# grantneale/kafka-lag-based-assignor

Measured on AMD Instinct MI355X. Metric: partition-assignments/sec (whole node), higher is better.
Workload: dtype int64

## Files before the change

### kafka_lag_based_assignor_amd/csrc/la_sort32.h

```cpp
#pragma once
#include <hip/hip_runtime.h>
#include <stdint.h>

#include "la_device.h"
#include "la_sort64.h"

#ifndef LA_SORT32_MED3
#define LA_SORT32_MED3 1
#endif

namespace la {

template <int J>
__device__ __forceinline__ uint32_t dir_vec() {
    const uint32_t lane = __builtin_amdgcn_mbcnt_hi(~0u, __builtin_amdgcn_mbcnt_lo(~0u, 0u));
    return (lane & (uint32_t)J) ? 0xFFFFFFFFu : 0u;
}

#if LA_SORT32_MED3
#define LA32_SAME_ASM(PADSTR, CTRL)                                             \
    asm volatile(PADSTR                                                         \
                 "v_mov_b32_dpp %1, %0 " CTRL LA_DPP_TAIL "\n\t"                \
                 "v_med3_u32 %0, %0, %1, %2"                                    \
                 : "+v"(x), "=&v"(t1)                                           \
                 : "v"(dir))

#define LA32_SAME_PADS(CTRL)                                      \
    do {                                                          \
        if constexpr (PAD == 0) LA32_SAME_ASM(LA_PAD0, CTRL);      \
        else if constexpr (PAD == 1) LA32_SAME_ASM(LA_PAD1, CTRL); \
        else LA32_SAME_ASM(LA_PAD2, CTRL);                         \
    } while (0)

template <int J, int PAD>
__device__ __forceinline__ void cmpx32_same_xor(uint32_t& x) {
    const uint32_t dir = dir_vec<J>();
    uint32_t t1;
    if constexpr (J == 1) LA32_SAME_PADS("quad_perm:[1,0,3,2]");
    else if constexpr (J == 2) LA32_SAME_PADS("quad_perm:[2,3,0,1]");
    else if constexpr (J == 8) LA32_SAME_PADS("row_ror:8");
    else if constexpr (J == 4) {
        uint32_t h;
        asm volatile(LA_PAD2
                     "v_mov_b32_dpp %2, %0 row_half_mirror" LA_DPP_TAIL "\n\t"
                     "s_nop 1\n\t"
                     "v_mov_b32_dpp %1, %2 quad_perm:[3,2,1,0]" LA_DPP_TAIL "\n\t"
                     "v_med3_u32 %0, %0, %1, %3"
                     : "+v"(x), "=&v"(t1), "=&v"(h)
                     : "v"(dir));
    } else {
        uint32_t b;
        if constexpr (J == 16)
            asm volatile(LA_PAD2 "v_mov_b32 %1, %0\n\ts_nop 1\n\tv_permlane16_swap_b32 %0, %1\n\t"
                         "v_med3_u32 %0, %0, %1, %2"
                         : "+v"(x), "=&v"(b) : "v"(dir));
        else
            asm volatile(LA_PAD2 "v_mov_b32 %1, %0\n\ts_nop 1\n\tv_permlane32_swap_b32 %0, %1\n\t"
                         "v_med3_u32 %0, %0, %1, %2"
                         : "+v"(x), "=&v"(b) : "v"(dir));
    }
}

template <int M, int PAD>
__device__ __forceinline__ void cmpx32_same_mirror(uint32_t& x) {
    if constexpr (M == 2) {
        cmpx32_same_xor<1, PAD>(x);
    } else if constexpr (M == 4 || M == 8 || M == 16) {
        const uint32_t dir = dir_vec<M / 2>();
        uint32_t t1;
        if constexpr (M == 4) LA32_SAME_PADS("quad_perm:[3,2,1,0]");
        else if constexpr (M == 8) LA32_SAME_PADS("row_half_mirror");
        else LA32_SAME_PADS("row_mirror");
    } else {
        asm volatile("s_nop 1" : "+v"(x));
        const uint32_t o = shfl_mirror<M>(x);
        const bool keep_min = (KeepMin<M / 2>::value >> __lane_id()) & 1;
        const uint32_t lo = o < x ? o : x, hi = o < x ? x : o;
        x = keep_min ? lo : hi;
        asm volatile("s_nop 1" : "+v"(x));
    }
}

#define LA32_CROSS_ASM(PADSTR, CTRL)                                            \
    asm volatile(PADSTR                                                         \
                 "v_mov_b32_dpp %2, %1 " CTRL LA_DPP_TAIL "\n\t"                \
                 "v_mov_b32_dpp %3, %0 " CTRL LA_DPP_TAIL "\n\t"                \
                 "v_med3_u32 %0, %0, %2, %4\n\t"                               \
                 "v_med3_u32 %1, %1, %3, %4"                                    \
                 : "+v"(r), "+v"(q), "=&v"(t1), "=&v"(t2)                        \
                 : "v"(dir))

#define LA32_CROSS_PADS(CTRL)                                      \
    do {                                                           \
        if constexpr (PAD == 0) LA32_CROSS_ASM(LA_PAD0, CTRL);      \
        else if constexpr (PAD == 1) LA32_CROSS_ASM(LA_PAD1, CTRL); \
        else LA32_CROSS_ASM(LA_PAD2, CTRL);                         \
    } while (0)

template <int M, int PAD>
__device__ __forceinline__ void cmpx32_cross_mirror(uint32_t& r, uint32_t& q) {
    if constexpr (M <= 16) {
        const uint32_t dir = dir_vec<M / 2>();
        uint32_t t1, t2;
        if constexpr (M == 2) LA32_CROSS_PADS("quad_perm:[1,0,3,2]");
        else if constexpr (M == 4) LA32_CROSS_PADS("quad_perm:[3,2,1,0]");
        else if constexpr (M == 8) LA32_CROSS_PADS("row_half_mirror");
        else LA32_CROSS_PADS("row_mirror");
    } else {
        const uint64_t keep = KeepMin<M / 2>::value;
        asm volatile("s_nop 1" : "+v"(r), "+v"(q));
        const uint32_t oq = shfl_mirror<M>(q), orr = shfl_mirror<M>(r);
        const bool keep_min = (keep >> __lane_id()) & 1;
        const uint32_t rl = oq < r ? oq : r, rh = oq < r ? r : oq;
        const uint32_t ql = orr < q ? orr : q, qh = orr < q ? q : orr;
        r = keep_min ? rl : rh;
        q = keep_min ? ql : qh;
        asm volatile("s_nop 1" : "+v"(r), "+v"(q));
    }
}

#else

#define LA32_SAME_ASM(PADSTR, CTRL)                                             \
    asm volatile(PADSTR                                                         \
                 "v_min_u32_dpp %1, %0, %0 " CTRL LA_DPP_TAIL "\n\t"              \
                 "v_max_u32_dpp %2, %0, %0 " CTRL LA_DPP_TAIL "\n\t"              \
                 "v_cndmask_b32_e64 %0, %2, %1, %3"                             \
                 : "+v"(x), "=&v"(t1), "=&v"(t2)                                 \
                 : "s"(keep))

#define LA32_SAME_PADS(CTRL)                                      \
    do {                                                          \
        if constexpr (PAD == 0) LA32_SAME_ASM(LA_PAD0, CTRL);      \
        else if constexpr (PAD == 1) LA32_SAME_ASM(LA_PAD1, CTRL); \
        else LA32_SAME_ASM(LA_PAD2, CTRL);                         \
    } while (0)

template <int J, int PAD>
__device__ __forceinline__ void cmpx32_same_xor(uint32_t& x) {
    const uint64_t keep = KeepMin<J>::value;
    uint32_t t1, t2;
    if constexpr (J == 1) LA32_SAME_PADS("quad_perm:[1,0,3,2]");
    else if constexpr (J == 2) LA32_SAME_PADS("quad_perm:[2,3,0,1]");
    else if constexpr (J == 8) LA32_SAME_PADS("row_ror:8");
    else if constexpr (J == 4) {
        uint32_t h;
        asm volatile(LA_PAD2
                     "v_mov_b32_dpp %3, %0 row_half_mirror" LA_DPP_TAIL "\n\t"
                     "s_nop 1\n\t"
                     "v_min_u32_dpp %1, %3, %0 quad_perm:[3,2,1,0]" LA_DPP_TAIL "\n\t"
                     "v_max_u32_dpp %2, %3, %0 quad_perm:[3,2,1,0]" LA_DPP_TAIL "\n\t"
                     "v_cndmask_b32_e64 %0, %2, %1, %4"
                     : "+v"(x), "=&v"(t1), "=&v"(t2), "=&v"(h)
                     : "s"(keep));
    } else {
        uint32_t b;
        if constexpr (J == 16)
            asm volatile(LA_PAD2 "v_mov_b32 %3, %0\n\ts_nop 1\n\tv_permlane16_swap_b32 %0, %3\n\t"
                         "v_min_u32 %1, %0, %3\n\tv_max_u32 %2, %0, %3\n\tv_cndmask_b32_e64 %0, %2, %1, %4"
                         : "+v"(x), "=&v"(t1), "=&v"(t2), "=&v"(b) : "s"(keep));
        else
            asm volatile(LA_PAD2 "v_mov_b32 %3, %0\n\ts_nop 1\n\tv_permlane32_swap_b32 %0, %3\n\t"
                         "v_min_u32 %1, %0, %3\n\tv_max_u32 %2, %0, %3\n\tv_cndmask_b32_e64 %0, %2, %1, %4"
                         : "+v"(x), "=&v"(t1), "=&v"(t2), "=&v"(b) : "s"(keep));
    }
}

template <int M, int PAD>
__device__ __forceinline__ void cmpx32_same_mirror(uint32_t& x) {
    if constexpr (M == 2) {
        cmpx32_same_xor<1, PAD>(x);
    } else if constexpr (M == 4 || M == 8 || M == 16) {
        const uint64_t keep = KeepMin<M / 2>::value;
        uint32_t t1, t2;
        if constexpr (M == 4) LA32_SAME_PADS("quad_perm:[3,2,1,0]");
        else if constexpr (M == 8) LA32_SAME_PADS("row_half_mirror");
        else LA32_SAME_PADS("row_mirror");
    } else {
        asm volatile("s_nop 1" : "+v"(x));
        const uint32_t o = shfl_mirror<M>(x);
        const bool keep_min = (KeepMin<M / 2>::value >> __lane_id()) & 1;
        const uint32_t lo = o < x ? o : x, hi = o < x ? x : o;
        x = keep_min ? lo : hi;
        asm volatile("s_nop 1" : "+v"(x));
    }
}

#define LA32_CROSS_ASM(PADSTR, CTRL)                                            \
    asm volatile(PADSTR                                                         \
                 "v_min_u32_dpp %2, %1, %0 " CTRL LA_DPP_TAIL "\n\t"              \
                 "v_max_u32_dpp %3, %1, %0 " CTRL LA_DPP_TAIL "\n\t"              \
                 "v_min_u32_dpp %4, %0, %1 " CTRL LA_DPP_TAIL "\n\t"              \
                 "v_max_u32_dpp %5, %0, %1 " CTRL LA_DPP_TAIL "\n\t"              \
                 "v_cndmask_b32_e64 %0, %3, %2, %6\n\t"                         \
                 "v_cndmask_b32_e64 %1, %5, %4, %6"                             \
                 : "+v"(r), "+v"(q), "=&v"(t1), "=&v"(t2), "=&v"(t3), "=&v"(t4)  \
                 : "s"(keep))

#define LA32_CROSS_PADS(CTRL)                                      \
    do {                                                           \
        if constexpr (PAD == 0) LA32_CROSS_ASM(LA_PAD0, CTRL);      \
        else if constexpr (PAD == 1) LA32_CROSS_ASM(LA_PAD1, CTRL); \
        else LA32_CROSS_ASM(LA_PAD2, CTRL);                         \
    } while (0)

template <int M, int PAD>
__device__ __forceinline__ void cmpx32_cross_mirror(uint32_t& r, uint32_t& q) {
    const uint64_t keep = KeepMin<M / 2>::value;
    if constexpr (M <= 16) {
        uint32_t t1, t2, t3, t4;
        if constexpr (M == 2) LA32_CROSS_PADS("quad_perm:[1,0,3,2]");
        else if constexpr (M == 4) LA32_CROSS_PADS("quad_perm:[3,2,1,0]");
        else if constexpr (M == 8) LA32_CROSS_PADS("row_half_mirror");
        else LA32_CROSS_PADS("row_mirror");
    } else {
        asm volatile("s_nop 1" : "+v"(r), "+v"(q));
        const uint32_t oq = shfl_mirror<M>(q), orr = shfl_mirror<M>(r);
        const bool keep_min = (keep >> __lane_id()) & 1;
        const uint32_t rl = oq < r ? oq : r, rh = oq < r ? r : oq;
        const uint32_t ql = orr < q ? orr : q, qh = orr < q ? q : orr;
        r = keep_min ? rl : rh;
        q = keep_min ? ql : qh;
        asm volatile("s_nop 1" : "+v"(r), "+v"(q));
    }
}

#endif

__device__ __forceinline__ void cmpx32_regs(uint32_t& a, uint32_t& b) {
    const uint32_t lo = a < b ? a : b, hi = a < b ? b : a;
    a = lo;
    b = hi;
}

template <int L, int E, int J>
__device__ __forceinline__ void clean32(uint32_t (&key)[E]) {
    if constexpr (J >= 1) {
        if constexpr (J >= E) {
            constexpr int PADN = (E <= 2) ? 2 : 0;
#pragma unroll
            for (int r = 0; r < E; ++r) cmpx32_same_xor<J / E, PADN>(key[r]);
        } else {
#pragma unroll
            for (int r = 0; r < E; ++r)
                if ((r & J) == 0) cmpx32_regs(key[r], key[r | J]);
        }
        clean32<L, E, J / 2>(key);
    }
}

template <int L, int E, int K>
__device__ __forceinline__ void merge32(uint32_t (&key)[E]) {
    if constexpr (K <= L * E) {
        if constexpr (K <= E) {
#pragma unroll
            for (int r = 0; r < E; ++r)
                if ((r & (K >> 1)) == 0) cmpx32_regs(key[r], key[r ^ (K - 1)]);
        } else {
            constexpr int M = K / E;
            if constexpr (E == 1) {
                cmpx32_same_mirror<M, 2>(key[0]);
            } else {
#pragma unroll
                for (int r = E / 2 - 1; r >= 0; --r) cmpx32_cross_mirror<M, 2>(key[r], key[E - 1 - r]);
            }
        }
        clean32<L, E, K / 4>(key);
        merge32<L, E, K * 2>(key);
    }
}

template <int L, int E>
__device__ __forceinline__ void bitonic_sort_tile_u32(uint32_t (&key)[E]) {
    merge32<L, E, 2>(key);
}

}
```

### kafka_lag_based_assignor_amd/csrc/la_sort64.h

```cpp
#pragma once
#include <hip/hip_runtime.h>
#include <stdint.h>

#include "la_device.h"

namespace la {

struct P64 {
    uint32_t lo, hi;
};

__device__ __forceinline__ P64 p64_from(uint64_t x) { P64 p; p.lo = (uint32_t)x; p.hi = (uint32_t)(x >> 32); return p; }
__device__ __forceinline__ uint64_t p64_value(const P64& p) { return ((uint64_t)p.hi << 32) | p.lo; }

template <int J>
struct KeepMin {
    static_assert(J == 1 || J == 2 || J == 4 || J == 8 || J == 16 || J == 32, "bad lane bit");
    static constexpr uint64_t value = J == 1 ? 0x5555555555555555ull : J == 2 ? 0x3333333333333333ull
                                    : J == 4 ? 0x0F0F0F0F0F0F0F0Full : J == 8 ? 0x00FF00FF00FF00FFull
                                    : J == 16 ? 0x0000FFFF0000FFFFull : 0x00000000FFFFFFFFull;
};

#define LA_DPP_TAIL " row_mask:0xf bank_mask:0xf"
#define LA_FIX_S(K) "s_xor_b64 vcc, vcc, " K "\n\t"
#define LA_FIX_V(T, K) "v_xor_b32 " T ", " K ", " T "\n\t" "v_cmp_gt_i32 vcc, 0, " T "\n\t"

template <int J>
__device__ __forceinline__ uint32_t keep_vec() {
    const uint32_t lane = __builtin_amdgcn_mbcnt_hi(~0u, __builtin_amdgcn_mbcnt_lo(~0u, 0u));
    return (lane & (uint32_t)J) ? 0u : 0xFFFFFFFFu;
}

#define LA_PAD0 ""
#define LA_PAD1 "s_nop 0\n\t"
#define LA_PAD2 "s_nop 1\n\t"

#define LA_SAME_ASM(PADSTR, CTRL, FIX, KC, KV)                                             \
    asm volatile(PADSTR                                                                    \
                 "v_sub_co_u32_dpp %2, vcc, %0, %0 " CTRL LA_DPP_TAIL "\n\t"                 \
                 "v_subb_co_u32_dpp %2, vcc, %1, %1, vcc " CTRL LA_DPP_TAIL "\n\t"           \
                 FIX                                                                       \
                 "v_cndmask_b32_dpp %0, %0, %0, vcc " CTRL LA_DPP_TAIL "\n\t"                \
                 "v_cndmask_b32_dpp %1, %1, %1, vcc " CTRL LA_DPP_TAIL                       \
                 : "+v"(r.lo), "+v"(r.hi), "=&v"(t)                                         \
                 : KC(KV)                                                                  \
                 : "vcc", "scc")
#define LA_SAME_VO(PADSTR, CTRL)                                                           \
    do {                                                                                   \
        if constexpr (VO) LA_SAME_ASM(PADSTR, CTRL, LA_FIX_V("%2", "%3"), "v", kvec);      \
        else LA_SAME_ASM(PADSTR, CTRL, LA_FIX_S("%3"), "s", keep);                         \
    } while (0)

#define LA_SAME_PADS(CTRL)                                  \
    do {                                                    \
        if constexpr (PAD == 0) LA_SAME_VO(LA_PAD0, CTRL);   \
        else if constexpr (PAD == 1) LA_SAME_VO(LA_PAD1, CTRL); \
        else LA_SAME_VO(LA_PAD2, CTRL);                      \
    } while (0)

#define LA_SAME_X4_ASM(PADSTR, FIX, KC, KV)                                                    \
    asm volatile(PADSTR                                                                        \
                 "v_mov_b32_dpp %2, %0 row_half_mirror" LA_DPP_TAIL "\n\t"                       \
                 "v_mov_b32_dpp %3, %1 row_half_mirror" LA_DPP_TAIL "\n\t"                       \
                 "s_nop 0\n\t"                                                                 \
                 "v_sub_co_u32_dpp %4, vcc, %2, %0 quad_perm:[3,2,1,0]" LA_DPP_TAIL "\n\t"       \
                 "v_subb_co_u32_dpp %4, vcc, %3, %1, vcc quad_perm:[3,2,1,0]" LA_DPP_TAIL "\n\t" \
                 FIX                                                                           \
                 "v_cndmask_b32_dpp %0, %2, %0, vcc quad_perm:[3,2,1,0]" LA_DPP_TAIL "\n\t"      \
                 "v_cndmask_b32_dpp %1, %3, %1, vcc quad_perm:[3,2,1,0]" LA_DPP_TAIL             \
                 : "+v"(r.lo), "+v"(r.hi), "=&v"(t), "=&v"(u), "=&v"(w)                          \
                 : KC(KV)                                                                      \
                 : "vcc", "scc")
#define LA_SAME_X4_VO(PADSTR)                                                              \
    do {                                                                                   \
        if constexpr (VO) LA_SAME_X4_ASM(PADSTR, LA_FIX_V("%4", "%5"), "v", kvec);         \
        else LA_SAME_X4_ASM(PADSTR, LA_FIX_S("%5"), "s", keep);                            \
    } while (0)

#define LA_SAME_SWAP_ASM(PADSTR, SWAP, FIX, KC, KV)          \
    asm volatile(PADSTR                                      \
                 "v_mov_b32 %2, %0\n\t"                      \
                 "v_mov_b32 %3, %1\n\t"                      \
                 "s_nop 1\n\t"                               \
                 SWAP " %0, %2\n\t"                          \
                 SWAP " %1, %3\n\t"                          \
                 "v_sub_co_u32 %4, vcc, %0, %2\n\t"          \
                 "v_subb_co_u32 %4, vcc, %1, %3, vcc\n\t"    \
                 FIX                                         \
// ... 12 lines not shown
__device__ __forceinline__ void cmpx_same_xor(P64& r) {
    [[maybe_unused]] const uint64_t keep = KeepMin<J>::value;
    [[maybe_unused]] const uint32_t kvec = keep_vec<J>();
    uint32_t t;
    if constexpr (J == 1) LA_SAME_PADS("quad_perm:[1,0,3,2]");
    else if constexpr (J == 2) LA_SAME_PADS("quad_perm:[2,3,0,1]");
    else if constexpr (J == 8) LA_SAME_PADS("row_ror:8");
    else if constexpr (J == 4) {
        uint32_t u, w;
        if constexpr (PAD == 0) LA_SAME_X4_VO(LA_PAD0);
        else if constexpr (PAD == 1) LA_SAME_X4_VO(LA_PAD1);
        else LA_SAME_X4_VO(LA_PAD2);
    } else {
        uint32_t u, w;
        if constexpr (J == 16) LA_SAME_SWAP_VO(LA_PAD2, "v_permlane16_swap_b32");
        else LA_SAME_SWAP_VO(LA_PAD2, "v_permlane32_swap_b32");
    }
}

#define LA_SELECT_ASM(FIX, KC, KV)                               \
    asm volatile("v_sub_co_u32 %2, vcc, %3, %0\n\t"              \
                 "v_subb_co_u32 %2, vcc, %4, %1, vcc\n\t"        \
                 FIX                                             \
                 "v_cndmask_b32 %0, %3, %0, vcc\n\t"             \
                 "v_cndmask_b32 %1, %4, %1, vcc"                 \
                 : "+v"(r.lo), "+v"(r.hi), "=&v"(t)              \
                 : "v"(o.lo), "v"(o.hi), KC(KV)                  \
                 : "vcc", "scc")
template <int J, bool VO = false>
__device__ __forceinline__ void select_minmax(P64& r, const P64& o) {
    uint32_t t;
    if constexpr (VO) {
        const uint32_t kvec = keep_vec<J>();
        LA_SELECT_ASM(LA_FIX_V("%2", "%5"), "v", kvec);
    } else {
        const uint64_t keep = KeepMin<J>::value;
        LA_SELECT_ASM(LA_FIX_S("%5"), "s", keep);
    }
}

template <int M, int PAD, bool VO = false>
__device__ __forceinline__ void cmpx_same_mirror(P64& r) {
    static_assert(M == 2 || M == 4 || M == 8 || M == 16 || M == 32 || M == 64, "bad mirror width");
    if constexpr (M == 2) {
        cmpx_same_xor<1, PAD, VO>(r);
    } else if constexpr (M == 4 || M == 8 || M == 16) {
        [[maybe_unused]] const uint64_t keep = KeepMin<M / 2>::value;
        [[maybe_unused]] const uint32_t kvec = keep_vec<M / 2>();
        uint32_t t;
        if constexpr (M == 4) LA_SAME_PADS("quad_perm:[3,2,1,0]");
        else if constexpr (M == 8) LA_SAME_PADS("row_half_mirror");
        else LA_SAME_PADS("row_mirror");
    } else {
        asm volatile("s_nop 1" : "+v"(r.lo), "+v"(r.hi));
        P64 o;
        o.lo = shfl_mirror<M>(r.lo);
        o.hi = shfl_mirror<M>(r.hi);
        select_minmax<M / 2, VO>(r, o);
    }
}

#define LA_CROSS_ASM(PADSTR, CTRL, FIX, KC, KV)                                             \
    asm volatile(PADSTR                                                                     \
                 "v_sub_co_u32_dpp %2, vcc, %0, %5 " CTRL LA_DPP_TAIL "\n\t"                  \
                 "v_subb_co_u32_dpp %2, vcc, %1, %6, vcc " CTRL LA_DPP_TAIL "\n\t"            \
                 FIX                                                                        \
                 "v_cndmask_b32_dpp %3, %0, %5, vcc " CTRL LA_DPP_TAIL "\n\t"                 \
                 "v_cndmask_b32_dpp %4, %1, %6, vcc " CTRL LA_DPP_TAIL "\n\t"                 \
                 "v_sub_co_u32_dpp %2, vcc, %5, %0 " CTRL LA_DPP_TAIL "\n\t"                  \
                 "v_subb_co_u32_dpp %2, vcc, %6, %1, vcc " CTRL LA_DPP_TAIL "\n\t"            \
                 FIX                                                                        \
                 "v_cndmask_b32_dpp %0, %5, %0, vcc " CTRL LA_DPP_TAIL "\n\t"                 \
                 "v_cndmask_b32_dpp %1, %6, %1, vcc " CTRL LA_DPP_TAIL                        \
                 : "+v"(q.lo), "+v"(q.hi), "=&v"(t), "=&v"(n.lo), "=&v"(n.hi)                       \
                 : "v"(r.lo), "v"(r.hi), KC(KV)                                             \
                 : "vcc", "scc")
#define LA_CROSS_VO(PADSTR, CTRL)                                                          \
    do {                                                                                   \
        if constexpr (VO) LA_CROSS_ASM(PADSTR, CTRL, LA_FIX_V("%2", "%7"), "v", kvec);     \
        else LA_CROSS_ASM(PADSTR, CTRL, LA_FIX_S("%7"), "s", keep);                        \
    } while (0)

#define LA_CROSS_PADS(CTRL)                                   \
    do {                                                      \
        if constexpr (PAD == 0) LA_CROSS_VO(LA_PAD0, CTRL);    \
        else if constexpr (PAD == 1) LA_CROSS_VO(LA_PAD1, CTRL); \
        else LA_CROSS_VO(LA_PAD2, CTRL);                       \
    } while (0)

template <int M, int PAD, bool VO = false>
__device__ __forceinline__ void cmpx_cross_mirror(P64& r, P64& q) {
    static_assert(M == 2 || M == 4 || M == 8 || M == 16 || M == 32 || M == 64, "bad mirror width");
    [[maybe_unused]] const uint64_t keep = KeepMin<M / 2>::value;
    [[maybe_unused]] const uint32_t kvec = keep_vec<M / 2>();
    if constexpr (M <= 16) {
        uint32_t t;
        P64 n;
        if constexpr (M == 2) LA_CROSS_PADS("quad_perm:[1,0,3,2]");
        else if constexpr (M == 4) LA_CROSS_PADS("quad_perm:[3,2,1,0]");
        else if constexpr (M == 8) LA_CROSS_PADS("row_half_mirror");
        else LA_CROSS_PADS("row_mirror");
        r = n;
    } else {
        asm volatile("s_nop 1" : "+v"(r.lo), "+v"(r.hi), "+v"(q.lo), "+v"(q.hi));
        P64 oq, orr;
        oq.lo = shfl_mirror<M>(q.lo); oq.hi = shfl_mirror<M>(q.hi);
        orr.lo = shfl_mirror<M>(r.lo); orr.hi = shfl_mirror<M>(r.hi);
        select_minmax<M / 2, VO>(r, oq);
        select_minmax<M / 2, VO>(q, orr);
    }
}

__device__ __forceinline__ void cmpx_regs_p64(P64& a, P64& b) {
    uint32_t t;
    P64 n;
    asm volatile("v_sub_co_u32 %2, vcc, %0, %5\n\t"
                 "v_subb_co_u32 %2, vcc, %1, %6, vcc\n\t"
                 "v_cndmask_b32 %3, %5, %0, vcc\n\t"
                 "v_cndmask_b32 %4, %6, %1, vcc\n\t"
                 "v_cndmask_b32 %0, %0, %5, vcc\n\t"
                 "v_cndmask_b32 %1, %1, %6, vcc"
                 : "+v"(b.lo), "+v"(b.hi), "=&v"(t), "=&v"(n.lo), "=&v"(n.hi)
                 : "v"(a.lo), "v"(a.hi)
                 : "vcc", "scc");
    a = n;
}


template <int L, int E, int J, bool FIRST, bool VO = false>
__device__ __forceinline__ void clean_p64(P64 (&rec)[E]) {
    if constexpr (J >= 1) {
        if constexpr (J >= E) {
            constexpr int PADN = (E <= 2) ? 1 : 0;
#pragma unroll
            for (int r = 0; r < E; ++r) cmpx_same_xor<J / E, PADN, VO>(rec[r]);
        } else {
#pragma unroll
            for (int r = 0; r < E; ++r)
                if ((r & J) == 0) cmpx_regs_p64(rec[r], rec[r | J]);
        }
        clean_p64<L, E, J / 2, false, VO>(rec);
    }
}

template <int L, int E, int K, bool FIRST, bool VO = false>
__device__ __forceinline__ void merge_p64(P64 (&rec)[E]) {
    if constexpr (K <= L * E) {
        if constexpr (K <= E) {
#pragma unroll
            for (int r = 0; r < E; ++r)
                if ((r & (K >> 1)) == 0) cmpx_regs_p64(rec[r], rec[r ^ (K - 1)]);
        } else {
            constexpr int M = K / E;
            if constexpr (E == 1) {
                cmpx_same_mirror<M, FIRST ? 2 : 1, VO>(rec[0]);
            } else {
                constexpr int PADN = FIRST ? 2 : ((E <= 2) ? 1 : 0);
#pragma unroll
                for (int r = E / 2 - 1; r >= 0; --r) cmpx_cross_mirror<M, PADN, VO>(rec[r], rec[E - 1 - r]);
            }
// ... 207 lines not shown
```

### kafka_lag_based_assignor_amd/csrc/la_wave_tile_impl.h

```cpp
#pragma once
#include "la_kernels.h"
#include "la_device.h"
#include "la_sort64.h"
#include "la_sort32.h"
#include "la_group_small.h"
#ifdef LA_LAB
#include <cstdio>
#include <cstdlib>
#endif

namespace la {

enum : int { kModeAuto = 0, kModeWide = 1, kModeArgmin = 2 };

#ifndef LA_ABLATE
#define LA_ABLATE 0
#endif
constexpr int kAblate = LA_ABLATE;
#ifndef LA_SKIP_SORTED_ROUNDS
#define LA_SKIP_SORTED_ROUNDS 1
#endif
constexpr bool kSkipSortedRounds = LA_SKIP_SORTED_ROUNDS != 0;
#ifndef LA_WPB
#define LA_WPB 4
#endif

template <int L, int E>
struct TileCfg {
    static constexpr int kGroupsPerWave = kWave / L;
    static constexpr int kWavesPerBlock = LA_WPB;
    static constexpr int kThreads = kWave * kWavesPerBlock;
    static constexpr int kTopicsPerBlock = kGroupsPerWave * kWavesPerBlock;
    static constexpr int kCap = L * E;
    static constexpr int kSlots = kCap + (kCap >> 3) + 1;
    static constexpr int kLog2Cap = (kCap <= 1) ? 0 : (31 - __builtin_clz(kCap - 1)) + 1;
};

__device__ __forceinline__ int slot_of(int s) { return s + (s >> 3); }

struct __attribute__((aligned(8))) I64x2 { int64_t x, y; };
struct __attribute__((aligned(4))) I32x2 { int32_t x, y; };

template <int L, int E>
__device__ __forceinline__ int load_index(int v, int gl) {
    if constexpr (E >= 2) return (v >> 1) * (2 * L) + 2 * gl + (v & 1);
    else return gl;
}

template <int E>
struct Raw {
    I64x2 en[(E + 1) / 2];
    I64x2 cm[(E + 1) / 2];
    I32x2 id[(E + 1) / 2];
};

template <typename IDX>
struct TopicDescT {
    IDX p0, c0;
    int P, C;
};
using TopicDesc = TopicDescT<int64_t>;

#ifndef LA_NT_LOADS
#define LA_NT_LOADS 1
#endif
template <typename V, typename T, typename IDX>
__device__ __forceinline__ V load_at(const T* base, IDX idx) {
    const V* p;
    if constexpr (sizeof(IDX) == 4)
        p = reinterpret_cast<const V*>(reinterpret_cast<const char*>(base) + (uint32_t)(idx * (uint32_t)sizeof(T)));
    else
        p = reinterpret_cast<const V*>(base + idx);
#if LA_NT_LOADS
    if constexpr (sizeof(V) == 16) {
        typedef long long LL2 __attribute__((ext_vector_type(2), aligned(8)));
// ... 10 lines not shown
    } else {
        return *p;
    }
#else
    return *p;
#endif
}

template <int L, int E, bool FULL = false, typename D>
__device__ __forceinline__ auto clamped_index(const TileArgs& a, const D& d, int v, int gl) {
    using IDX = decltype(d.p0);
    const IDX g = d.p0 + (IDX)load_index<L, E>(v, gl);
    if constexpr (FULL) return g;
    const IDX hi = (IDX)(a.n_total - (E >= 2 ? 2 : 1));
    return g < hi ? g : hi;
}

template <int L, int E, bool FULL = false, typename D>
__device__ __forceinline__ void issue_loads(const TileArgs& a, const D& d, int gl, Raw<E>& raw) {
    if constexpr (kAblate == 2) return;
    constexpr int NP = (E + 1) / 2;
    const int64_t* src_en = a.lag ? a.lag : a.end;
    if (!a.lag) {
#pragma unroll
        for (int k = 0; k < NP; ++k) {
            const auto g = clamped_index<L, E, FULL>(a, d, 2 * k, gl);
            if constexpr (E >= 2) raw.cm[k] = load_at<I64x2>(a.committed, g);
            else { raw.cm[k].x = load_at<int64_t>(a.committed, g); raw.cm[k].y = 0; }
        }
    } else {
#pragma unroll
        for (int k = 0; k < NP; ++k) raw.cm[k].x = raw.cm[k].y = 0;
    }
#pragma unroll
    for (int k = 0; k < NP; ++k) {
        const auto g = clamped_index<L, E, FULL>(a, d, 2 * k, gl);
        if constexpr (E >= 2) {
            raw.en[k] = load_at<I64x2>(src_en, g);
            raw.id[k] = load_at<I32x2>(a.pid, g);
        } else {
            raw.en[k].x = load_at<int64_t>(src_en, g); raw.en[k].y = 0;
            raw.id[k].x = load_at<int32_t>(a.pid, g); raw.id[k].y = 0;
        }
    }
}

template <int L, int E>
__device__ __forceinline__ bool second_stage_needed(const TileArgs& a) {
    return !a.lag && !a.reset_latest && a.begin;
}

template <int L, int E, bool FULL = false, typename D>
__device__ __forceinline__ void issue_begin_loads(const TileArgs& a, const D& d, int gl, Raw<E>& raw) {
    if constexpr (kAblate == 2) return;
    constexpr int NP = (E + 1) / 2;
    if (!second_stage_needed<L, E>(a)) return;
    {
        bool any = false;
#pragma unroll
        for (int k = 0; k < NP; ++k) any |= (raw.cm[k].x < 0) | (E >= 2 && raw.cm[k].y < 0);
        if (__builtin_amdgcn_ballot_w64(any) == 0 && !(a.flags & kTileAlwaysStage2)) return;
    }
#pragma unroll
    for (int k = 0; k < NP; ++k) {
        const auto g = clamped_index<L, E, FULL>(a, d, 2 * k, gl);
        using G = decltype(g);
        const bool nx = raw.cm[k].x < 0;
        if constexpr (E >= 2) {
            const bool ny = raw.cm[k].y < 0;
            const I64x2 bv = load_at<I64x2>(a.begin, (nx | ny) ? g : (G)0);
            raw.cm[k].x = nx ? bv.x : raw.cm[k].x;
            raw.cm[k].y = ny ? bv.y : raw.cm[k].y;
        } else {
            const int64_t vx = a.begin[nx ? g : (G)0];
            raw.cm[k].x = nx ? vx : raw.cm[k].x;
        }
    }
}

template <int L, int E, bool FULL = false, typename D>
__device__ __forceinline__ void finish_lags(const TileArgs& a, const D& d, int gl, const Raw<E>& raw,
                                            int64_t (&lag)[E], int32_t (&pid)[E]) {
    const bool latest = a.reset_latest != 0;
    if constexpr (kAblate == 2) {
#pragma unroll
        for (int v = 0; v < E; ++v) {
            const uint32_t h = ((uint32_t)d.p0 + (uint32_t)(v * L + gl)) * 2654435761u;
            lag[v] = (int64_t)(h >> 2) + a.reset_latest;
            pid[v] = (int32_t)((v * L + gl) * 77 + 13) & (L * E - 1);
        }
        return;
    }
    constexpr int NP = (E + 1) / 2;
    const bool cm_is_next = second_stage_needed<L, E>(a);
    auto lag_of = [&](int64_t en, int64_t cm) -> int64_t {
        if (a.lag) return en;
        if (cm_is_next) { const int64_t dlt = (int64_t)((uint64_t)en - (uint64_t)cm); return dlt > 0 ? dlt : 0; }
        return partition_lag(0, en, cm, latest);
    };
#pragma unroll
    for (int k = 0; k < NP; ++k) {
        const int e = load_index<L, E>(2 * k, gl);
        const bool shifted = !FULL && (E >= 2) && (d.p0 + (decltype(d.p0))e == (decltype(d.p0))(a.n_total - 1));
        const int64_t en_x = shifted ? raw.en[k].y : raw.en[k].x;
        const int64_t cm_x = shifted ? raw.cm[k].y : raw.cm[k].x;
        pid[2 * k] = shifted ? raw.id[k].y : raw.id[k].x;
        lag[2 * k] = lag_of(en_x, cm_x);
        if constexpr (E >= 2) {
            pid[2 * k + 1] = raw.id[k].y;
            lag[2 * k + 1] = lag_of(raw.en[k].y, raw.cm[k].y);
        }
    }
    if constexpr (FULL) return;
#pragma unroll
    for (int v = 0; v < E; ++v) {
        const bool valid = load_index<L, E>(v, gl) < d.P;
        lag[v] = valid ? lag[v] : 0;
        pid[v] = valid ? pid[v] : 0;
    }
}

template <int L, int E, bool FULL = false>
__device__ __forceinline__ void pack_records(int P, int gl, const int64_t (&lag)[E], const int32_t (&pid)[E], int sh,
                                             uint64_t lag_max, P64 (&rec)[E]) {
#pragma unroll
    for (int v = 0; v < E; ++v) {
        const int e = load_index<L, E>(v, gl);
        rec[v] = p64_from((FULL || e < P) ? (((lag_max - (uint64_t)lag[v]) << sh) | (uint32_t)pid[v]) : ~0ull);
    }
}

template <int L, int E, bool FULL = false>
__device__ __forceinline__ void sort_into_slice(uint64_t* slice, int gl, P64 (&rec)[E], int lbw, int sh) {
    using Cfg = TileCfg<L, E>;
    if constexpr (kAblate == 1 || kAblate == 4) {
#pragma unroll
        for (int r = 0; r < E; ++r) slice[slot_of(gl * E + r)] = p64_value(rec[r]);
        return;
    }
#ifdef LA_TILE_SORT64
    bitonic_sort_tile_p64<L, E>(rec);
#pragma unroll
    for (int r = 0; r < E; ++r) slice[slot_of(gl * E + r)] = p64_value(rec[r]);
    return;
#endif
    const bool by_id = sh <= Cfg::kLog2Cap;
    const int idx_bits = by_id ? sh : Cfg::kLog2Cap;
    const uint32_t idx_mask = (1u << idx_bits) - 1;
    const int top_bits = by_id ? lbw : lbw + sh;
    const int keep = 31 - idx_bits;
    const int drop = (by_id ? sh : 0) + (top_bits > keep ? top_bits - keep : 0);
    uint32_t key[E];
    if (by_id && drop == sh) {
#pragma unroll
        for (int v = 0; v < E; ++v) key[v] = (!FULL && rec[v].hi == 0xFFFFFFFFu) ? 0xFFFFFFFFu : rec[v].lo;
        bitonic_sort_tile_u32<L, E>(key);
#pragma unroll
        for (int r = 0; r < E; ++r)
            slice[slot_of(gl * E + r)] = (!FULL && key[r] == 0xFFFFFFFFu) ? ~0ull : (uint64_t)key[r];
        return;
    }
#pragma unroll
    for (int v = 0; v < E; ++v) {
        const uint64_t r = p64_value(rec[v]);
        const bool valid = FULL || r != ~0ull;
        const uint32_t idx = by_id ? ((uint32_t)r & idx_mask) : (uint32_t)load_index<L, E>(v, gl);
        if (valid) slice[slot_of((int)idx)] = r;
        key[v] = valid ? (((uint32_t)(r >> drop) << idx_bits) | idx) : 0xFFFFFFFFu;
    }
    wave_lds_fence();
    bitonic_sort_tile_u32<L, E>(key);

    P64 got[E];
#pragma unroll
    for (int r = 0; r < E; ++r) {
        const uint64_t x = slice[slot_of((int)(key[r] & idx_mask))];
        got[r] = p64_from((!FULL && key[r] == 0xFFFFFFFFu) ? ~0ull : x);
    }
    bool bad = false;
#pragma unroll
    for (int r = 0; r + 1 < E; ++r) {
        const uint64_t x = p64_value(got[r]), y = p64_value(got[r + 1]);
        bad |= (x >= y) && (FULL || y != ~0ull);
    }
    {
        const uint64_t x = p64_value(got[E - 1]);
        const uint64_t y = p64_of_next_lane(got[0]);
        bad |= (gl != L - 1) && (x >= y) && (FULL || y != ~0ull);
    }
    wave_lds_fence();
    if (__builtin_amdgcn_ballot_w64(bad) != 0) {
        bitonic_sort_tile_p64<L, E>(rec);
#pragma unroll
        for (int r = 0; r < E; ++r) slice[slot_of(gl * E + r)] = p64_value(rec[r]);
    } else {
#pragma unroll
        for (int r = 0; r < E; ++r) slice[slot_of(gl * E + r)] = p64_value(got[r]);
    }
}

template <int L, int LC>
__device__ __forceinline__ void greedy_rounds_tile(P64& bin, uint64_t* slice, int P, int C, int gl, int sh,
                                                   uint64_t lag_max, uint32_t pid_mask, int max_rounds) {
    for (int q = 0; q < max_rounds; ++q) {
        const uint64_t desc = q >= 1 ? lane_descents_p64<L>(bin) : 0;
        if (q >= 1 && kSkipSortedRounds && desc == 0) {
        } else if (q == 1) {
            bool mirrored = false;
            if constexpr (LC == L) {
                const uint64_t mine = p64_value(bin);
                const uint64_t prev = p64_of_prev_lane(bin);
                const bool bad = (C != L) || (gl > 0 && !((prev >> 6) > (mine >> 6)));
                if (__builtin_amdgcn_ballot_w64(bad) == 0) {
                    bin.lo = shfl_mirror<L>(bin.lo);
                    bin.hi = shfl_mirror<L>(bin.hi);
                    mirrored = true;
                }
            }
            if (!mirrored) bitonic_sort_lanes_p64<LC>(bin);
        } else if (q > 1) {
            settle_lanes_p64<L, LC>(bin, desc);
        }
        const int s = q * C + gl;
        if (gl < C && s < P) {
            const uint64_t r = slice[slot_of(s)];
            const uint64_t nb = p64_value(bin) + ((lag_max - (r >> sh)) << 6);
            bin = p64_from(nb);
            slice[slot_of(s)] = ((uint64_t)(bin.lo & 63u) << 32) | ((uint32_t)r & pid_mask);
        }
    }
}

__device__ __forceinline__ uint32_t wire_element(int32_t id, int32_t rank, int id_bits, uint32_t limit, bool& bad) {
    const uint32_t r1 = (uint32_t)rank + 1u;
    const uint32_t w = (r1 << id_bits) | (uint32_t)id;
    bad |= ((uint32_t)id >> id_bits) != 0 || r1 >= limit;
    return w;
}

template <int L, int E, bool FULL = false, bool WIRE = false, typename IDX>
__device__ __forceinline__ void assign_packed(const TileArgs& a, uint64_t* slice, int32_t* rank_tab, IDX p0,
                                              IDX c0, int P, int C, int gl, int sh, uint64_t lag_max,
                                              int32_t my_rank) {
    const uint32_t pid_mask = (uint32_t)((1ull << sh) - 1);

    if (gl < C) rank_tab[gl] = my_rank;
    wave_lds_fence();

    P64 bin = p64_from((gl < C) ? (uint64_t)gl : ~0ull);
    const int rounds = (C > 0) ? (P + C - 1) / C : 0;
    int max_rounds = wave_max_of_groups_i32<L>(rounds);
    if constexpr (kAblate == 1 || kAblate == 3) max_rounds = 0;
    if constexpr (kAblate >= 10) max_rounds = max_rounds < kAblate - 10 ? max_rounds : kAblate - 10;
    const int c_max = wave_max_of_groups_i32<L>(C);
    bool done = false;
    if constexpr (L > 4) if (!done && c_max <= 4) { greedy_rounds_tile<L, 4>(bin, slice, P, C, gl, sh, lag_max, pid_mask, max_rounds); done = true; }
    if constexpr (L > 8) if (!done && c_max <= 8) { greedy_rounds_tile<L, 8>(bin, slice, P, C, gl, sh, lag_max, pid_mask, max_rounds); done = true; }
    if constexpr (L > 16) if (!done && c_max <= 16) { greedy_rounds_tile<L, 16>(bin, slice, P, C, gl, sh, lag_max, pid_mask, max_rounds); done = true; }
    if constexpr (L > 32) if (!done && c_max <= 32) { greedy_rounds_tile<L, 32>(bin, slice, P, C, gl, sh, lag_max, pid_mask, max_rounds); done = true; }
    if (!done) greedy_rounds_tile<L, L>(bin, slice, P, C, gl, sh, lag_max, pid_mask, max_rounds);
    wave_lds_fence();

    if (a.out_total && gl < C) a.out_total[c0 + (bin.lo & 63u)] = (int64_t)(p64_value(bin) >> 6);
    if constexpr (WIRE) {
        const int id_bits = a.wire_id_bits;
        const bool two = a.wire_bytes == 2;
        const int rank_bits = (two ? 16 : 32) - id_bits;
        const uint32_t limit = rank_bits >= 32 ? 0xFFFFFFFFu : (1u << rank_bits);
        bool bad = false;
        if constexpr (E >= 4) {
#pragma unroll
            for (int k = 0; k < E / 4; ++k) {
                const int s0 = k * 4 * L + 4 * gl;
                uint32_t wv[4];
#pragma unroll
                for (int i = 0; i < 4; ++i) {
                    const uint64_t w = slice[slot_of(s0 + i)];
                    bool b1 = false;
                    wv[i] = wire_element((int32_t)((uint32_t)w & pid_mask), (C > 0) ? rank_tab[(uint32_t)(w >> 32) & 63u] : -1, id_bits, limit,
                                         b1);
                    bad |= b1 && (FULL || s0 + i < P);
                }
                if (FULL || s0 + 3 < P) {
                    if (two) {
                        typedef uint32_t U32x2w __attribute__((ext_vector_type(2), aligned(2)));
                        const U32x2w v = {wv[0] | (wv[1] << 16), wv[2] | (wv[3] << 16)};
                        __builtin_nontemporal_store(v, reinterpret_cast<U32x2w*>(reinterpret_cast<uint16_t*>(a.out_wire) + p0 + s0));
                    } else {
                        typedef uint32_t U32x4w __attribute__((ext_vector_type(4), aligned(4)));
                        const U32x4w v = {wv[0], wv[1], wv[2], wv[3]};
                        __builtin_nontemporal_store(v, reinterpret_cast<U32x4w*>(reinterpret_cast<uint32_t*>(a.out_wire) + p0 + s0));
                    }
                } else {
#pragma unroll
                    for (int i = 0; i < 4; ++i)
                        if (s0 + i < P) {
                            if (two) reinterpret_cast<uint16_t*>(a.out_wire)[p0 + s0 + i] = (uint16_t)wv[i];
                            else reinterpret_cast<uint32_t*>(a.out_wire)[p0 + s0 + i] = wv[i];
                        }
                }
            }
        } else {
#pragma unroll
            for (int v = 0; v < E; ++v) {
                const int s = v * L + gl;
// ... 178 lines not shown

template <int L, int E, typename IDX = int64_t>
__device__ __forceinline__ TopicDescT<IDX> make_desc(const TileArgs& a, const DescWords& w, int gl) {
    using Cfg = TileCfg<L, E>;
    TopicDescT<IDX> d;
    d.p0 = (IDX)w.p0;
    d.c0 = (IDX)w.c0;
    const int64_t Pl = w.p1 - w.p0, Cl = w.c1 - w.c0;
    const bool bad = Pl > Cfg::kCap || Cl > L || Pl < 0 || Cl < 0;
    if (w.exists && bad && gl == 0 && !(a.flags & kTileSkipOversize)) atomicOr(a.status, kStatusShape);
    d.P = (w.exists && !bad) ? (int)Pl : 0;
    d.C = (w.exists && !bad) ? (int)Cl : 0;
    return d;
}

template <int L, int E, typename IDX = int64_t>
__device__ __forceinline__ TopicDescT<IDX> load_desc(const TileArgs& a, int64_t t, int64_t n_tiles, int grp, int gl) {
    return make_desc<L, E, IDX>(a, fetch_desc<L, E>(a, t, n_tiles, grp), gl);
}

template <int L, int E, typename IDX = int64_t>
__device__ __forceinline__ TopicDescT<IDX> load_desc_uniform(const TileArgs& a, int64_t t, int64_t n_tiles, int grp, int gl) {
    constexpr int G = TileCfg<L, E>::kGroupsPerWave;
    if (!a.topic_list && (t + 1) * G <= a.n_topics)
        return make_desc<L, E, IDX>(a, fetch_desc_uniform<L, E>(a, t, grp), gl);
    return make_desc<L, E, IDX>(a, fetch_desc<L, E>(a, t, n_tiles, grp), gl);
}

template <int L, int E, typename IDX, bool INLINE_WIDE, bool FULL, bool WIRE = false>
__device__ __forceinline__ void packed_tile(const TileArgs& a, const TopicDescT<IDX>& cur, uint64_t* slice, int32_t* rank_tab,
                                            int64_t tile, int gl, int lane) {
    using Cfg = TileCfg<L, E>;
    Raw<E> raw;
    issue_loads<L, E, FULL>(a, cur, gl, raw);
    int32_t my_rank = 0;
    if constexpr (kAblate != 2) {
        const IDX want = cur.c0 + (IDX)gl, last = (IDX)(a.k_total > 0 ? a.k_total - 1 : 0);
        if (a.k_total > 0) my_rank = load_at<int32_t>(a.cons_rank, want < last ? want : last);
    }
    issue_begin_loads<L, E, FULL>(a, cur, gl, raw);

    P64 rec[E];
    int sh, lbw;
    bool fits;
    uint64_t lag_max;
    int64_t lag[E];
    int32_t pid[E];
    {
        finish_lags<L, E, FULL>(a, cur, gl, raw, lag, pid);
        uint32_t id_or = 0;
        uint64_t lag_or = 0;
#pragma unroll
        for (int v = 0; v < E; ++v) { id_or |= (uint32_t)pid[v]; lag_or |= (uint64_t)lag[v]; }
        id_or = wave_or_u32_uniform(id_or);
        sh = 32 - __builtin_clz(id_or | 1u);
        lbw = bits_of_or_u64(wave_or_u32_uniform((uint32_t)(lag_or >> 32)), wave_or_u32_uniform((uint32_t)lag_or));
        int lim = 63 - sh;
        if (lim > 57 - Cfg::kLog2Cap) lim = 57 - Cfg::kLog2Cap;
        fits = sh < 32 && lbw <= lim;
        lag_max = lbw >= 64 ? ~0ull : (((uint64_t)1 << lbw) - 1);
        if (fits) pack_records<L, E, FULL>(cur.P, gl, lag, pid, sh, lag_max, rec);
    }
    if (fits) {
        sort_into_slice<L, E, FULL>(slice, gl, rec, lbw, sh);
        assign_packed<L, E, FULL, WIRE>(a, slice, rank_tab, cur.p0, cur.c0, cur.P, cur.C, gl, sh, lag_max, my_rank);
    } else if constexpr (INLINE_WIDE) {
        assign_wide<L, E, false>(a, slice, (int64_t)cur.p0, (int64_t)cur.c0, cur.P, cur.C, gl, lag, pid);
    } else if (lane == 0) {
        if (a.flags & kTileNoDefer) atomicOr(a.status, kStatusBounds);
        else a.defer_list[atomicAdd(a.defer_count, 1)] = (int32_t)tile;
    }
}

__device__ __forceinline__ void tile_tail(const TileTail& t, const uint32_t* status) {
    __shared__ uint32_t s_start[kTailGroupM];
    __shared__ int32_t s_in[7 * kSmallGroupN];
    __shared__ uint32_t s_wsum[LA_WPB];
    __shared__ uint32_t s_turn, s_last;
    __threadfence_system();
    __syncthreads();
    if (threadIdx.x == 0) {
        const uint32_t done = __hip_atomic_fetch_add(t.counter, 1u, __ATOMIC_ACQ_REL, __HIP_MEMORY_SCOPE_AGENT);
        s_last = done == gridDim.x - 1 ? 1u : 0u;
    }
    __syncthreads();
    if (!s_last) return;
    __builtin_amdgcn_fence(__ATOMIC_ACQUIRE, "agent");
    if (threadIdx.x == 0) __hip_atomic_store(t.counter, 0u, __ATOMIC_RELAXED, __HIP_MEMORY_SCOPE_AGENT);
    if (t.member_off)
        group_small_body_staged<kWave * LA_WPB, kTailGroupM>(t.n, t.n_members, t.n_topics, t.part_off, t.out_pid, t.out_rank,
                                                             t.member_off, t.grouped_topic, t.grouped_partition, nullptr, s_start,
                                                             s_wsum, &s_turn, s_in, s_in + kSmallGroupN, s_in + 2 * kSmallGroupN,
                                                             s_in + 3 * kSmallGroupN, s_in + 4 * kSmallGroupN,
                                                             reinterpret_cast<uint32_t*>(s_in + 5 * kSmallGroupN),
                                                             reinterpret_cast<uint32_t*>(s_in + 6 * kSmallGroupN));
    __threadfence_system();
    __syncthreads();
    if (threadIdx.x == 0) {
        const uint32_t st = __hip_atomic_load(status, __ATOMIC_RELAXED, __HIP_MEMORY_SCOPE_AGENT);
        __hip_atomic_store(t.fin_flag, 0x80000000u | st, __ATOMIC_RELEASE, __HIP_MEMORY_SCOPE_SYSTEM);
    }
}

#ifdef LA_WPE
#define LA_WPE_ATTR __attribute__((amdgpu_waves_per_eu(LA_WPE, LA_WPE)))
#else
#define LA_WPE_ATTR
#endif
template <int L, int E, typename IDX, bool INLINE_WIDE, bool WIRE = false>
// ... 154 lines not shown
```

Baseline: 200.0 billion.

## Replace shuffle-based 32/64-lane mirrors with DPP+permlane swaps and pair-batched med3

Replaces the generic shfl_mirror path for row-crossing (32/64-lane) bitonic mirror compare-exchanges with inline DPP row_mirror plus v_permlane16/32_swap sequences, using v_med3 with a direction vector. It adds a two-pair variant that interleaves two compare-exchanges to hide swap latency, and applies the same mirror to the 64-bit sort path and the greedy-round reversal. It also skips the high-word wave OR reduction when no lane has nonzero upper lag bits, and adds new ablation modes. The aim is to avoid ds_bpermute/LDS-backed shuffles and their waits, at the cost of hand-tuned nop padding that must be correct for hazards.

```diff
diff --git a/kafka_lag_based_assignor_amd/csrc/la_sort32.h b/kafka_lag_based_assignor_amd/csrc/la_sort32.h
--- a/kafka_lag_based_assignor_amd/csrc/la_sort32.h
+++ b/kafka_lag_based_assignor_amd/csrc/la_sort32.h
@@ -61,6 +61,83 @@
     }
 }
 
+#define LA32_SMIRROR32_ASM                                     \
+    "v_mov_b32_dpp %1, %0 row_mirror" LA_DPP_TAIL "\n\t"       \
+    "v_mov_b32_dpp %2, %0 row_mirror" LA_DPP_TAIL "\n\t"       \
+    "s_nop 1\n\t"                                              \
+    "v_permlane16_swap_b32 %1, %2\n\t"                         \
+    "s_nop 1\n\t"                                              \
+    "v_permlane16_swap_b32 %2, %1\n\t"                         \
+    "v_med3_u32 %0, %0, %2, %3"
+#define LA32_SMIRROR64_ASM                                     \
+    "v_mov_b32_dpp %1, %0 row_mirror" LA_DPP_TAIL "\n\t"       \
+    "v_mov_b32_dpp %2, %0 row_mirror" LA_DPP_TAIL "\n\t"       \
+    "s_nop 1\n\t"                                              \
+    "v_permlane16_swap_b32 %1, %2\n\t"                         \
+    "s_nop 1\n\t"                                              \
+    "v_permlane16_swap_b32 %2, %1\n\t"                         \
+    "s_nop 1\n\t"                                              \
+    "v_permlane32_swap_b32 %2, %1\n\t"                         \
+    "s_nop 1\n\t"                                              \
+    "v_permlane32_swap_b32 %1, %2\n\t"                         \
+    "v_med3_u32 %0, %0, %1, %3"
+#define LA32_XMIRROR32_ASM                                     \
+    "v_mov_b32_dpp %2, %1 row_mirror" LA_DPP_TAIL "\n\t"       \
+    "v_mov_b32_dpp %3, %0 row_mirror" LA_DPP_TAIL "\n\t"       \
+    "s_nop 1\n\t"                                              \
+    "v_permlane16_swap_b32 %2, %3\n\t"                         \
+    "s_nop 1\n\t"                                              \
+    "v_permlane16_swap_b32 %3, %2\n\t"                         \
+    "v_med3_u32 %0, %0, %3, %4\n\t"                            \
+    "v_med3_u32 %1, %1, %2, %4"
+#define LA32_XMIRROR64_ASM                                     \
+    "v_mov_b32_dpp %2, %1 row_mirror" LA_DPP_TAIL "\n\t"       \
+    "v_mov_b32_dpp %3, %0 row_mirror" LA_DPP_TAIL "\n\t"       \
+    "s_nop 1\n\t"                                              \
+    "v_permlane16_swap_b32 %2, %3\n\t"                         \
+    "s_nop 1\n\t"                                              \
+    "v_permlane16_swap_b32 %3, %2\n\t"                         \
+    "s_nop 1\n\t"                                              \
+    "v_permlane32_swap_b32 %3, %2\n\t"                         \
+    "s_nop 1\n\t"                                              \
+    "v_permlane32_swap_b32 %2, %3\n\t"                         \
+    "v_med3_u32 %0, %0, %2, %4\n\t"                            \
+    "v_med3_u32 %1, %1, %3, %4"
+#define LA32_XMIRROR32_X2_ASM                                  \
+    "v_mov_b32_dpp %4, %1 row_mirror" LA_DPP_TAIL "\n\t"       \
+    "v_mov_b32_dpp %5, %0 row_mirror" LA_DPP_TAIL "\n\t"       \
+    "v_mov_b32_dpp %6, %3 row_mirror" LA_DPP_TAIL "\n\t"       \
+    "v_mov_b32_dpp %7, %2 row_mirror" LA_DPP_TAIL "\n\t"       \
+    "v_permlane16_swap_b32 %4, %5\n\t"                         \
+    "s_nop 0\n\t"                                              \
+    "v_permlane16_swap_b32 %6, %7\n\t"                         \
+    "v_permlane16_swap_b32 %5, %4\n\t"                         \
+    "v_med3_u32 %0, %0, %5, %8\n\t"                            \
+    "v_med3_u32 %1, %1, %4, %8\n\t"                            \
+    "v_permlane16_swap_b32 %7, %6\n\t"                         \
+    "v_med3_u32 %2, %2, %7, %8\n\t"                            \
+    "v_med3_u32 %3, %3, %6, %8"
+#define LA32_XMIRROR64_X2_ASM                                  \
+    "v_mov_b32_dpp %4, %1 row_mirror" LA_DPP_TAIL "\n\t"       \
+    "v_mov_b32_dpp %5, %0 row_mirror" LA_DPP_TAIL "\n\t"       \
+    "v_mov_b32_dpp %6, %3 row_mirror" LA_DPP_TAIL "\n\t"       \
+    "v_mov_b32_dpp %7, %2 row_mirror" LA_DPP_TAIL "\n\t"       \
+    "v_permlane16_swap_b32 %4, %5\n\t"                         \
+    "s_nop 0\n\t"                                              \
+    "v_permlane16_swap_b32 %6, %7\n\t"                         \
+    "v_permlane16_swap_b32 %5, %4\n\t"                         \
+    "s_nop 0\n\t"                                              \
+    "v_permlane16_swap_b32 %7, %6\n\t"                         \
+    "v_permlane32_swap_b32 %5, %4\n\t"                         \
+    "s_nop 0\n\t"                                              \
+    "v_permlane32_swap_b32 %7, %6\n\t"                         \
+    "v_permlane32_swap_b32 %4, %5\n\t"                         \
+    "v_med3_u32 %0, %0, %4, %8\n\t"                            \
+    "v_med3_u32 %1, %1, %5, %8\n\t"                            \
+    "v_permlane32_swap_b32 %6, %7\n\t"                         \
+    "v_med3_u32 %2, %2, %6, %8\n\t"                            \
+    "v_med3_u32 %3, %3, %7, %8"
+
 template <int M, int PAD>
 __device__ __forceinline__ void cmpx32_same_mirror(uint32_t& x) {
     if constexpr (M == 2) {
@@ -72,12 +149,10 @@
         else if constexpr (M == 8) LA32_SAME_PADS("row_half_mirror");
         else LA32_SAME_PADS("row_mirror");
     } else {
-        asm volatile("s_nop 1" : "+v"(x));
-        const uint32_t o = shfl_mirror<M>(x);
-        const bool keep_min = (KeepMin<M / 2>::value >> __lane_id()) & 1;
-        const uint32_t lo = o < x ? o : x, hi = o < x ? x : o;
-        x = keep_min ? lo : hi;
-        asm volatile("s_nop 1" : "+v"(x));
+        const uint32_t dir = dir_vec<M / 2>();
+        uint32_t t1, t2;
+        if constexpr (M == 32) asm volatile(LA_PAD2 LA32_SMIRROR32_ASM : "+v"(x), "=&v"(t1), "=&v"(t2) : "v"(dir));
+        else asm volatile(LA_PAD2 LA32_SMIRROR64_ASM : "+v"(x), "=&v"(t1), "=&v"(t2) : "v"(dir));
     }
 }
 
@@ -107,17 +182,26 @@
         else if constexpr (M == 8) LA32_CROSS_PADS("row_half_mirror");
         else LA32_CROSS_PADS("row_mirror");
     } else {
-        const uint64_t keep = KeepMin<M / 2>::value;
-        asm volatile("s_nop 1" : "+v"(r), "+v"(q));
-        const uint32_t oq = shfl_mirror<M>(q), orr = shfl_mirror<M>(r);
-        const bool keep_min = (keep >> __lane_id()) & 1;
-        const uint32_t rl = oq < r ? oq : r, rh = oq < r ? r : oq;
-        const uint32_t ql = orr < q ? orr : q, qh = orr < q ? q : orr;
-        r = keep_min ? rl : rh;
-        q = keep_min ? ql : qh;
-        asm volatile("s_nop 1" : "+v"(r), "+v"(q));
-    }
-}
+        const uint32_t dir = dir_vec<M / 2>();
+        uint32_t tq, tr;
+        if constexpr (M == 32) asm volatile(LA_PAD2 LA32_XMIRROR32_ASM : "+v"(r), "+v"(q), "=&v"(tq), "=&v"(tr) : "v"(dir));
+        else asm volatile(LA_PAD2 LA32_XMIRROR64_ASM : "+v"(r), "+v"(q), "=&v"(tq), "=&v"(tr) : "v"(dir));
+    }
+}
+
+template <int M>
+__device__ __forceinline__ void cmpx32_cross_mirror2(uint32_t& r0, uint32_t& q0, uint32_t& r1, uint32_t& q1) {
+    static_assert(M == 32 || M == 64, "row-crossing mirrors only");
+    const uint32_t dir = dir_vec<M / 2>();
+    uint32_t tq0, tr0, tq1, tr1;
+    if constexpr (M == 32)
+        asm volatile(LA_PAD2 LA32_XMIRROR32_X2_ASM
+                     : "+v"(r0), "+v"(q0), "+v"(r1), "+v"(q1), "=&v"(tq0), "=&v"(tr0), "=&v"(tq1), "=&v"(tr1) : "v"(dir));
+    else
+        asm volatile(LA_PAD2 LA32_XMIRROR64_X2_ASM
+                     : "+v"(r0), "+v"(q0), "+v"(r1), "+v"(q1), "=&v"(tq0), "=&v"(tr0), "=&v"(tq1), "=&v"(tr1) : "v"(dir));
+}
+constexpr bool kMirrorTwoPairs = true;
 
 #else
 
@@ -224,6 +308,12 @@
         asm volatile("s_nop 1" : "+v"(r), "+v"(q));
     }
 }
+template <int M>
+__device__ __forceinline__ void cmpx32_cross_mirror2(uint32_t& r0, uint32_t& q0, uint32_t& r1, uint32_t& q1) {
+    cmpx32_cross_mirror<M, 2>(r0, q0);
+    cmpx32_cross_mirror<M, 2>(r1, q1);
+}
+constexpr bool kMirrorTwoPairs = false;
 
 #endif
 
@@ -260,6 +350,10 @@
             constexpr int M = K / E;
             if constexpr (E == 1) {
                 cmpx32_same_mirror<M, 2>(key[0]);
+            } else if constexpr (kMirrorTwoPairs && M > 16 && E >= 4) {
+#pragma unroll
+                for (int r = E / 2 - 1; r >= 1; r -= 2)
+                    cmpx32_cross_mirror2<M>(key[r], key[E - 1 - r], key[r - 1], key[E - r]);
             } else {
 #pragma unroll
                 for (int r = E / 2 - 1; r >= 0; --r) cmpx32_cross_mirror<M, 2>(key[r], key[E - 1 - r]);
diff --git a/kafka_lag_based_assignor_amd/csrc/la_sort64.h b/kafka_lag_based_assignor_amd/csrc/la_sort64.h
--- a/kafka_lag_based_assignor_amd/csrc/la_sort64.h
+++ b/kafka_lag_based_assignor_amd/csrc/la_sort64.h
@@ -34,6 +34,66 @@
 #define LA_PAD0 ""
 #define LA_PAD1 "s_nop 0\n\t"
 #define LA_PAD2 "s_nop 1\n\t"
+
+#define LA_MIRROR_PAIR32_ASM                                   \
+    "v_mov_b32_dpp %0, %2 row_mirror" LA_DPP_TAIL "\n\t"       \
+    "v_mov_b32_dpp %1, %3 row_mirror" LA_DPP_TAIL "\n\t"       \
+    "s_nop 1\n\t"                                              \
+    "v_permlane16_swap_b32 %0, %1\n\t"                         \
+    "s_nop 1\n\t"                                              \
+    "v_permlane16_swap_b32 %1, %0"
+#define LA_MIRROR_PAIR64_ASM                                   \
+    LA_MIRROR_PAIR32_ASM "\n\t"                                \
+    "s_nop 1\n\t"                                              \
+    "v_permlane32_swap_b32 %1, %0\n\t"                         \
+    "s_nop 1\n\t"                                              \
+    "v_permlane32_swap_b32 %0, %1"
+#define LA_MIRROR_QUAD32_ASM                                   \
+    "v_mov_b32_dpp %0, %4 row_mirror" LA_DPP_TAIL "\n\t"       \
+    "v_mov_b32_dpp %1, %5 row_mirror" LA_DPP_TAIL "\n\t"       \
+    "v_mov_b32_dpp %2, %6 row_mirror" LA_DPP_TAIL "\n\t"       \
+    "v_mov_b32_dpp %3, %7 row_mirror" LA_DPP_TAIL "\n\t"       \
+    "v_permlane16_swap_b32 %0, %1\n\t"                         \
+    "s_nop 0\n\t"                                              \
+    "v_permlane16_swap_b32 %2, %3\n\t"                         \
+    "v_permlane16_swap_b32 %1, %0\n\t"                         \
+    "s_nop 0\n\t"                                              \
+    "v_permlane16_swap_b32 %3, %2"
+#define LA_MIRROR_QUAD64_ASM                                   \
+    LA_MIRROR_QUAD32_ASM "\n\t"                                \
+    "v_permlane32_swap_b32 %1, %0\n\t"                         \
+    "s_nop 0\n\t"                                              \
+    "v_permlane32_swap_b32 %3, %2\n\t"                         \
+    "v_permlane32_swap_b32 %0, %1\n\t"                         \
+    "s_nop 0\n\t"                                              \
+    "v_permlane32_swap_b32 %2, %3"
+
+template <int M>
+__device__ __forceinline__ void mirror_pair_u32(uint32_t a, uint32_t b, uint32_t& oa, uint32_t& ob) {
+    static_assert(M == 32 || M == 64, "row-crossing mirrors only");
+    uint32_t ta, tb;
+    if constexpr (M == 32) {
+        asm volatile(LA_PAD2 LA_MIRROR_PAIR32_ASM : "=&v"(ta), "=&v"(tb) : "v"(a), "v"(b));
+        oa = tb; ob = ta;
+    } else {
+        asm volatile(LA_PAD2 LA_MIRROR_PAIR64_ASM : "=&v"(ta), "=&v"(tb) : "v"(a), "v"(b));
+        oa = ta; ob = tb;
+    }
+}
+
+template <int M>
+__device__ __forceinline__ void mirror_quad_u32(uint32_t a, uint32_t b, uint32_t c, uint32_t d, uint32_t& oa, uint32_t& ob,
+                                                uint32_t& oc, uint32_t& od) {
+    static_assert(M == 32 || M == 64, "row-crossing mirrors only");
+    uint32_t ta, tb, tc, td;
+    if constexpr (M == 32) {
+        asm volatile(LA_PAD2 LA_MIRROR_QUAD32_ASM : "=&v"(ta), "=&v"(tb), "=&v"(tc), "=&v"(td) : "v"(a), "v"(b), "v"(c), "v"(d));
+        oa = tb; ob = ta; oc = td; od = tc;
+    } else {
+        asm volatile(LA_PAD2 LA_MIRROR_QUAD64_ASM : "=&v"(ta), "=&v"(tb), "=&v"(tc), "=&v"(td) : "v"(a), "v"(b), "v"(c), "v"(d));
+        oa = ta; ob = tb; oc = tc; od = td;
+    }
+}
 
 #define LA_SAME_ASM(PADSTR, CTRL, FIX, KC, KV)                                             \
     asm volatile(PADSTR                                                                    \
@@ -152,10 +212,8 @@
         else if constexpr (M == 8) LA_SAME_PADS("row_half_mirror");
         else LA_SAME_PADS("row_mirror");
     } else {
-        asm volatile("s_nop 1" : "+v"(r.lo), "+v"(r.hi));
         P64 o;
-        o.lo = shfl_mirror<M>(r.lo);
-        o.hi = shfl_mirror<M>(r.hi);
+        mirror_pair_u32<M>(r.lo, r.hi, o.lo, o.hi);
         select_minmax<M / 2, VO>(r, o);
     }
 }
@@ -202,10 +260,8 @@
         else LA_CROSS_PADS("row_mirror");
         r = n;
     } else {
-        asm volatile("s_nop 1" : "+v"(r.lo), "+v"(r.hi), "+v"(q.lo), "+v"(q.hi));
         P64 oq, orr;
-        oq.lo = shfl_mirror<M>(q.lo); oq.hi = shfl_mirror<M>(q.hi);
-        orr.lo = shfl_mirror<M>(r.lo); orr.hi = shfl_mirror<M>(r.hi);
+        mirror_quad_u32<M>(q.lo, r.lo, q.hi, r.hi, oq.lo, orr.lo, oq.hi, orr.hi);
         select_minmax<M / 2, VO>(r, oq);
         select_minmax<M / 2, VO>(q, orr);
     }
diff --git a/kafka_lag_based_assignor_amd/csrc/la_wave_tile_impl.h b/kafka_lag_based_assignor_amd/csrc/la_wave_tile_impl.h
--- a/kafka_lag_based_assignor_amd/csrc/la_wave_tile_impl.h
+++ b/kafka_lag_based_assignor_amd/csrc/la_wave_tile_impl.h
@@ -17,10 +17,16 @@
 #define LA_ABLATE 0
 #endif
 constexpr int kAblate = LA_ABLATE;
+constexpr bool kAblateNoSort = kAblate == 1 || kAblate == 4 || kAblate == 5 || kAblate == 6;
+constexpr bool kAblateNoGreedy = kAblate == 1 || kAblate == 3 || kAblate == 5 || kAblate == 6;
 #ifndef LA_SKIP_SORTED_ROUNDS
 #define LA_SKIP_SORTED_ROUNDS 1
 #endif
 constexpr bool kSkipSortedRounds = LA_SKIP_SORTED_ROUNDS != 0;
+#ifndef LA_SKIP_ZERO_HIGH_OR
+#define LA_SKIP_ZERO_HIGH_OR 1
+#endif
+constexpr bool kSkipZeroHighOr = LA_SKIP_ZERO_HIGH_OR != 0;
 #ifndef LA_WPB
 #define LA_WPB 4
 #endif
@@ -137,7 +143,7 @@
 
 template <int L, int E, bool FULL = false, typename D>
 __device__ __forceinline__ void issue_begin_loads(const TileArgs& a, const D& d, int gl, Raw<E>& raw) {
-    if constexpr (kAblate == 2) return;
+    if constexpr (kAblate == 2 || kAblate == 5) return;
     constexpr int NP = (E + 1) / 2;
     if (!second_stage_needed<L, E>(a)) return;
     {
@@ -218,7 +224,7 @@
 template <int L, int E, bool FULL = false>
 __device__ __forceinline__ void sort_into_slice(uint64_t* slice, int gl, P64 (&rec)[E], int lbw, int sh) {
     using Cfg = TileCfg<L, E>;
-    if constexpr (kAblate == 1 || kAblate == 4) {
+    if constexpr (kAblateNoSort) {
 #pragma unroll
         for (int r = 0; r < E; ++r) slice[slot_of(gl * E + r)] = p64_value(rec[r]);
         return;
@@ -297,8 +303,12 @@
                 const uint64_t prev = p64_of_prev_lane(bin);
                 const bool bad = (C != L) || (gl > 0 && !((prev >> 6) > (mine >> 6)));
                 if (__builtin_amdgcn_ballot_w64(bad) == 0) {
-                    bin.lo = shfl_mirror<L>(bin.lo);
-                    bin.hi = shfl_mirror<L>(bin.hi);
+                    if constexpr (L > 16) {
+                        mirror_pair_u32<L>(bin.lo, bin.hi, bin.lo, bin.hi);
+                    } else {
+                        bin.lo = shfl_mirror<L>(bin.lo);
+                        bin.hi = shfl_mirror<L>(bin.hi);
+                    }
                     mirrored = true;
                 }
             }
@@ -335,7 +345,7 @@
     P64 bin = p64_from((gl < C) ? (uint64_t)gl : ~0ull);
     const int rounds = (C > 0) ? (P + C - 1) / C : 0;
     int max_rounds = wave_max_of_groups_i32<L>(rounds);
-    if constexpr (kAblate == 1 || kAblate == 3) max_rounds = 0;
+    if constexpr (kAblateNoGreedy) max_rounds = 0;
     if constexpr (kAblate >= 10) max_rounds = max_rounds < kAblate - 10 ? max_rounds : kAblate - 10;
     const int c_max = wave_max_of_groups_i32<L>(C);
     bool done = false;
@@ -620,9 +630,11 @@
         uint64_t lag_or = 0;
 #pragma unroll
         for (int v = 0; v < E; ++v) { id_or |= (uint32_t)pid[v]; lag_or |= (uint64_t)lag[v]; }
-        id_or = wave_or_u32_uniform(id_or);
+        id_or = kAblate == 6 ? 255u : wave_or_u32_uniform(id_or);
         sh = 32 - __builtin_clz(id_or | 1u);
-        lbw = bits_of_or_u64(wave_or_u32_uniform((uint32_t)(lag_or >> 32)), wave_or_u32_uniform((uint32_t)lag_or));
+        const uint32_t lag_hi = (uint32_t)(lag_or >> 32);
+        const uint32_t hi_or = (!kSkipZeroHighOr || __builtin_amdgcn_ballot_w64(lag_hi != 0) != 0) ? wave_or_u32_uniform(lag_hi) : 0u;
+        lbw = kAblate == 6 ? 30 : bits_of_or_u64(hi_or, wave_or_u32_uniform((uint32_t)lag_or));
         int lim = 63 - sh;
         if (lim > 57 - Cfg::kLog2Cap) lim = 57 - Cfg::kLog2Cap;
         fits = sh < 32 && lbw <= lim;
```

Result: no change. 198.7 billion, median of 3 (-0.7%).
